# RobotVisionHKA/LiFCal

Measured on AMD Instinct MI355X. Metric: micro-image obs/sec through Jacobian+Schur at 1M obs, higher is better.
Workload: dtype f64; 1 GPU; metric_web: 334 frames, 24720 points, 999994 micro-image observations, window 10, config 0xf06 (2 radial + tangential, mlCenterAdj, Cauchy(0.5), refine poses+points); lens_selection=reference generator (lifcal_mla_project), obs_per_gpu=999994, n_reduced=2021, deterministic=False

## Files before the change

lifcal_amd/csrc/kernels.hpp:

```cpp
#pragma once
#include <hip/hip_runtime.h>
#include <stdint.h>

#include <type_traits>

#include "../../include/lifcal_ba.h"
#include "device_model.hpp"
#include "lm_step.hpp"

namespace lifcal {

constexpr uint32_t DET_NF_MAX = 20;
constexpr int SCAL_COST = 0, SCAL_BAD_U = 1, SCAL_GMAX0 = 2, SCAL_N = 2 + 64;
constexpr int ST_GTD = 0, ST_DDD = 1, ST_STEP2 = 2, ST_X2 = 3, ST_CAND_COST = 4, ST_CHOL_FAIL = 5, ST_GMAX_RED = 6, ST_DIR = 7, ST_N = 8;

struct TileSet { uint32_t n_tiles; const uint32_t *tile_row0, *slot_pt, *slot_fr, *slot_cnt, *ell_lens; const double *ell_u, *ell_v; };

struct Dev {
  uint32_t F, P, Q, NA, bw, nc, n_tiles, n_slots, n_lenses, n_red, ld, M_local, n_owned;
  uint32_t n_radial, tangential, adj, robust, use_poses, use_points, rank, world;
  uint32_t fixed_mask;
  double spx, spy, scale, loss_scale;
  double lm_min, lm_max;
  double *cam, *views, *pts, *cam_c, *views_c, *pts_c;
  const double *lower, *upper;
  CamConsts *camc, *camc_c;
  double *ft, *ft_c, *lt, *lt_c;
  const uint32_t *tile_row0, *slot_pt, *slot_fr, *slot_cnt, *ell_lens;
  const double *ell_u, *ell_v;
  const int32_t* promoted;
  const uint32_t* promoted_ids;
  double* panel_g;
  const uint32_t *pt_slot0, *pt_nslots, *owned;
  const uint8_t* frame_live;
  double *ptacc;
  double *Uinv, *lamP, *sigP;
  double *Wv;
  double *Av;
  const uint8_t* pt_special;
  const uint32_t *gid_fr, *slot_gid;
  uint32_t n_blocks, v2_nfmax, n_special;
  const uint32_t *blk_pass0, *blk_flo, *blk_nf, *pass_pt0, *pass_np, *pass_gid0, *pass_ng, *v2_points, *v2_ptinfo, *v2_slot, *v2_tile_row0, *v2_lens, *v2f_pt, *v2_passpt, *v2_gidx;
  const double *v2_u, *v2_v;
  uint32_t n_fwg;
  const uint32_t *fwg_blk, *fwg_pass0, *blk_pt0;
  const float *v2_du, *v2_dv;
  float* ltf;
  double* ltw;
  uint32_t deterministic, det_stride;
  double *det_slab, *det_slots;
  uint32_t* det_turn;
  const uint32_t* special_owned;
  const uint32_t *c_i, *c_j, *my_cons, *pt_cons0, *pt_cons_list; const double *c_dist, *c_sigma;
  double* Wpart;
  double *Sband, *Sarrow, *rhsacc, *gB, *hdiag, *scal;
  double *sig_red, *lam_red, *delta_red, *Linv;
  double* lm;
  double* step;
  double* dP;
  unsigned long long* dbg;
};

LIFCAL_DEV double lm_radius(const Dev& d, double arg) { return arg < 0.0 ? d.lm[LM_RADIUS] : arg; }

LIFCAL_DEV double* s_addr(const Dev& d, uint32_t row, uint32_t col) {
  if (row < 6 * d.F) {
    const uint32_t f = row / 6, i = row % 6, fc = col / 6, j = col % 6;
    return d.Sband + ((size_t)f * (d.bw + 1) + (f - fc)) * 36 + i * 6 + j;
  }
  return d.Sarrow + (size_t)(row - 6 * d.F) * d.ld + col;
}
LIFCAL_DEV void s_add(const Dev& d, uint32_t row, uint32_t col, double v) {
  if (row >= col) atomicAdd(s_addr(d, row, col), v); else atomicAdd(s_addr(d, col, row), v);
}

LIFCAL_DEV double wave_sum(double v) {
#pragma unroll
  for (int m = 32; m >= 1; m >>= 1) v += __shfl_xor(v, m, 64);
  return v;
}

LIFCAL_DEV void det_turn_wait(const Dev& d, uint32_t which, uint32_t my) {
  uint32_t* turn = d.det_turn + which;
  const uint64_t t0 = __builtin_amdgcn_s_memrealtime();
  for (;;) {
    const uint32_t v = (uint32_t)__builtin_amdgcn_readfirstlane((int)__hip_atomic_load(turn, __ATOMIC_ACQUIRE, __HIP_MEMORY_SCOPE_AGENT));
    if (v == my) break;
    __builtin_amdgcn_s_sleep(16);
// ... 237 lines not shown
  {
    int t = 0;
#pragma unroll
    for (int i = 0; i < NC; ++i) {
#pragma unroll
      for (int j = 0; j <= i; ++j) {
        const double s = wave_sum(cc[t]);
        if (lane == (uint32_t)(t & 63)) { atomicAdd(d.Sarrow + (size_t)(camrow + i) * d.ld + camcol + j, s); if (i == j) atomicAdd(d.hdiag + camcol + i, s); }
        ++t;
      }
    }
#pragma unroll
    for (int i = 0; i < NC; ++i) { const double s = wave_sum(gc[i]); if (lane == (uint32_t)i) atomicAdd(d.gB + camcol + i, s); }
    const double s = wave_sum(cost);
    if (lane == 63) atomicAdd(d.scal + SCAL_COST, s);
  }
  if (d.deterministic) det_turn_pass(d, 0, wave);
}

LIFCAL_DEV double finalize_column(const Dev& d, uint32_t t, double radius) {
  const uint32_t F6 = 6 * d.F, A0 = F6 + 3 * d.Q;
  double* diag = s_addr(d, t, t);
  double* rhs = d.Sarrow + (size_t)d.NA * d.ld;
  const uint32_t fl = t < F6 ? (uint32_t)d.frame_live[t / 6] : 1u;
  const double ch = t >= A0 ? d.camc->chm[t - A0] : 1.0;
  const double s = d.sig_red[t], h = d.hdiag[t], g = d.gB[t], ra = d.rhsacc[t], dg = *diag;
  const double rad = lm_radius(d, radius);
  const bool live = t < F6 ? (d.use_poses && fl) : ch != 0.0;
  const double lam = live ? fmin(fmax(h * s * s, d.lm_min), d.lm_max) / (rad * s * s) : 0.0;
  d.lam_red[t] = lam;
  *diag = live ? dg + lam : 1.0;
  rhs[t] = live ? -g + ra : 0.0;
  return fabs(g);
}

}
#include "sweep2.hpp"
#include "sweep3.hpp"
#include "sweep4.hpp"
namespace lifcal {

__global__ void k_constraints(Dev d, int cost_only, const double* pts, double* cost_out) {
  for (uint32_t t = blockIdx.x * blockDim.x + threadIdx.x; t < d.M_local; t += gridDim.x * blockDim.x) {
  const uint32_t c = d.my_cons[t];
  const uint32_t pi = d.c_i[c], pj = d.c_j[c];
  const double* Pi = pts + 3 * (size_t)pi; const double* Pj = pts + 3 * (size_t)pj;
  const double dx = Pi[0] - Pj[0], dy = Pi[1] - Pj[1], dz = Pi[2] - Pj[2];
  const double n = sqrt(dx * dx + dy * dy + dz * dz);
  const double is = 1.0 / (d.c_sigma[c] + 0.000001);
  const double r = (n - d.c_dist[c]) * is;
  atomicAdd(cost_out, 0.5 * r * r);
  if (cost_only) continue;
  const double in = is / n;
  const double Ji[3] = {dx * in, dy * in, dz * in};
  const uint32_t F6 = 6 * d.F;
  const int32_t qi = d.promoted[pi], qj = d.promoted[pj];
  const uint32_t cj = F6 + 3 * (uint32_t)qj;
  for (int a = 0; a < 3; ++a) {
    for (int b = 0; b <= a; ++b) s_add(d, cj + a, cj + b, Ji[a] * Ji[b]);
    atomicAdd(d.hdiag + cj + a, Ji[a] * Ji[a]);
    atomicAdd(d.gB + cj + a, -Ji[a] * r);
  }
  if (qi < 0) {
    double* acc = d.ptacc + (size_t)pi * 36;
    atomicAdd(acc + 0, Ji[0] * Ji[0]); atomicAdd(acc + 1, Ji[1] * Ji[0]); atomicAdd(acc + 2, Ji[2] * Ji[0]);
    atomicAdd(acc + 3, Ji[1] * Ji[1]); atomicAdd(acc + 4, Ji[2] * Ji[1]); atomicAdd(acc + 5, Ji[2] * Ji[2]);
// ... 279 lines not shown
  const uint32_t e = blockIdx.x, lane = threadIdx.x;
  const uint32_t camrow = 3 * d.Q, camcol = 6 * d.F + 3 * d.Q;
  uint32_t off; double* dst; bool is_max = false;
  if (e < NCC) {
    if (mode != 0) return;
    uint32_t i = 0; while ((i + 1) * (i + 2) / 2 <= e) ++i;
    off = lay.off_cc + e; dst = d.Sarrow + (size_t)(camrow + i) * d.ld + camcol + (e - i * (i + 1) / 2);
  } else if (e < NCC + 3 * NC) {
    const uint32_t q = e - NCC, w = q / NC, j = q % NC;
    if (mode != 0 && w != 1) return;
    off = lay.off_vec + w * vlen + 6 * NFm + j; dst = (w == 0 ? d.gB : (w == 1 ? d.hdiag : d.rhsacc)) + camcol + j;
  } else {
    if (mode != 0) return;
    const uint32_t q = e - NCC - 3 * NC;
    off = lay.off_fr + q; is_max = q == 2;
    dst = d.scal + (q == 0 ? SCAL_COST : (q == 1 ? SCAL_BAD_U : SCAL_GMAX0 + d.rank));
  }
  double v = 0.0;
  for (uint32_t b = lane; b < nB; b += 64) { const double x = d.det_slab[(size_t)b * d.det_stride + off]; v = is_max ? fmax(v, x) : v + x; }
#pragma unroll
  for (int m = 32; m >= 1; m >>= 1) { const double o = __shfl_xor(v, m, 64); v = is_max ? fmax(v, o) : v + o; }
  if (lane == 0) { if (is_max) *dst = fmax(*dst, v); else *dst += v; }
}

__global__ void k_det_sum(const double* slots, uint32_t n_wg, uint32_t K, double* dst) {
  const uint32_t k = threadIdx.x;
  if (k >= K) return;
  double s = 0.0;
  for (uint32_t g = 0; g < n_wg; ++g) s += slots[(size_t)g * K + k];
  dst[k] += s;
}

constexpr uint32_t FIN_ZERO_PER_WG = 256 * 4;
__global__ void k_finalize(Dev d, double radius, uint32_t n_fin, double* zero, uint32_t n_zero) {
  if (blockIdx.x >= n_fin) {
    const uint32_t n_threads = (gridDim.x - n_fin) * blockDim.x, t0 = (blockIdx.x - n_fin) * blockDim.x + threadIdx.x;
    const uint32_t odd = (uint32_t)(((uintptr_t)zero >> 3) & 1u), head = odd < n_zero ? odd : n_zero;
    const uint32_t n2 = (n_zero - head) / 2;
    double2* z2 = reinterpret_cast<double2*>(zero + head);
    for (uint32_t i = t0; i < n2; i += n_threads) z2[i] = double2{0.0, 0.0};
    if (t0 == 0 && head) zero[0] = 0.0;
    if (t0 == 0 && head + 2 * n2 < n_zero) zero[n_zero - 1] = 0.0;
    return;
  }
  const uint32_t t = blockIdx.x * blockDim.x + threadIdx.x;
  if (t == 0) d.lm[LM_T0] = (double)__builtin_amdgcn_s_memrealtime();
  double g = 0.0;
  if (t < d.n_red) g = finalize_column(d, t, radius);
#pragma unroll
  for (int m = 32; m >= 1; m >>= 1) g = fmax(g, __shfl_xor(g, m, 64));
  if ((threadIdx.x & 63u) == 0) atomicMax((unsigned long long*)(d.step + ST_GMAX_RED), (unsigned long long)__double_as_longlong(g));
}

__global__ __launch_bounds__(1024) void k_band_chol(Dev d) {
  extern __shared__ __attribute__((aligned(16))) double smem[];
  double* Ld = smem; double* Li = smem + 36; double* failp = smem + 72;
  double* panel = d.panel_g ? d.panel_g : smem + 80;
  const uint32_t tid = threadIdx.x, nt = blockDim.x;
  const uint32_t F = d.F, bw = d.bw, NAx = d.NA + 1, ld = d.ld;
  if (tid == 0) *failp = 0.0;
  __syncthreads();
  for (uint32_t j = 0; j < F; ++j) {
    double* Sjj = d.Sband + (size_t)j * (bw + 1) * 36;
    if (tid == 0) {
      double L[6][6];
      for (int a = 0; a < 6; ++a) for (int b = 0; b <= a; ++b) L[a][b] = Sjj[a * 6 + b];
      bool ok = true;
      for (int c = 0; c < 6; ++c) {
        double dg = L[c][c];
        for (int k = 0; k < c; ++k) dg -= L[c][k] * L[c][k];
        if (!(dg > 0.0)) { ok = false; dg = 1.0; }
        dg = sqrt(dg); L[c][c] = dg;
        for (int r = c + 1; r < 6; ++r) { double s = L[r][c]; for (int k = 0; k < c; ++k) s -= L[r][k] * L[c][k]; L[r][c] = s / dg; }
      }
      if (!ok) *failp = 1.0;
      double I[6][6];
      for (int c = 0; c < 6; ++c) {
        for (int r = 0; r < 6; ++r) I[r][c] = 0.0;
        I[c][c] = 1.0 / L[c][c];
        for (int r = c + 1; r < 6; ++r) { double s = 0.0; for (int k = c; k < r; ++k) s -= L[r][k] * I[k][c]; I[r][c] = s / L[r][r]; }
      }
      for (int a = 0; a < 6; ++a) for (int b = 0; b < 6; ++b) { Ld[a * 6 + b] = (b <= a) ? L[a][b] : 0.0; Li[a * 6 + b] = (b <= a) ? I[a][b] : 0.0; }
      for (int a = 0; a < 6; ++a) for (int b = 0; b <= a; ++b) Sjj[a * 6 + b] = L[a][b];
      for (int k = 0; k < 36; ++k) d.Linv[(size_t)j * 36 + k] = Li[k];
    }
// ... 491 lines not shown
```

lifcal_amd/csrc/lifcal_ba.hip:

```cpp
#include <hip/hip_runtime.h>
#include <hip/hip_ext.h>

#include <dlfcn.h>

#include <chrono>
#include <cmath>
#include <cstdio>
#include <cstdlib>
#include <cstring>
#include <limits>
#include <mutex>
#include <string>
#include <vector>

#include "../../include/lifcal_ba.h"
#include "kernels.hpp"
#include "plan.hpp"
#include "linesearch.hpp"
#include "sweep_state.hpp"

using namespace lifcal;

static_assert(lifcal::DET_NF_MAX == lifcal::Plan::NF_MAX, "k_det_reduce searches the covering blocks of a frame inside Plan::NF_MAX frames");
static_assert(lifcal::Plan::PASS_GROUPS == 256, "k_det_reduce / k_det_reduce_all read the window layout of 256-lane passes (V2Lds(nf, true, 256))");
// ... 115 lines not shown
  std::vector<hipEvent_t> prof_events; uint32_t prof_cap = 0, prof_used = 0, prof_seen = 0, prof_stride = 1; bool prof_on = false, prof_closed = false;
  hipEvent_t prof_span0 = nullptr, prof_span1 = nullptr;
  hipEvent_t prof_ev(int which) { return prof_events[(size_t)prof_used * 6 + which]; }
  bool prof_in_span() const { return prof_on && prof_seen < prof_cap; }
  bool prof_active() const { return prof_in_span() && prof_seen % prof_stride == 0; }
};

namespace {

template <class T>
int dev_alloc(lifcal_ba_handle* h, T** p, size_t n) {
  *p = nullptr;
  if (n == 0) n = 1;
  HIP_TRY(hipMalloc((void**)p, n * sizeof(T)));
  h->allocs.push_back(*p);
  h->bytes += n * sizeof(T);
  return 0;
}
template <class T, class A>
int dev_upload(lifcal_ba_handle* h, T** p, const std::vector<T, A>& v) {
  if (int rc = dev_alloc(h, p, v.size())) return rc;
  if (!v.empty()) HIP_TRY(hipMemcpy(*p, v.data(), v.size() * sizeof(T), hipMemcpyHostToDevice));
  return 0;
}

int do_allreduce(lifcal_ba_handle* h, double* buf, size_t count) {
  if (h->opt.world_size <= 1) return 0;
  if (h->hook) { if (h->hook(h->hook_ctx, buf, count, (void*)h->stream) != 0) { g_last_error = "all-reduce hook failed"; return LIFCAL_BA_ERR_COMM; } return 0; }
  if (h->comm) { if (g_rccl.AllReduce(buf, buf, count, kNcclFloat64, kNcclSum, h->comm, h->stream) != 0) { g_last_error = "ncclAllReduce failed"; return LIFCAL_BA_ERR_COMM; } return 0; }
  g_last_error = "world_size > 1 but neither lifcal_ba_set_allreduce nor lifcal_ba_comm_init_rccl was called";
  return LIFCAL_BA_ERR_COMM;
}

int exchange_reduced(lifcal_ba_handle* h) {
  if (h->opt.world_size <= 1 && !h->force_exchange) return 0;
  const bool have_gather = h->ghook ? (h->hook != nullptr) : (h->hook == nullptr && h->comm != nullptr);
  if (!h->xch_ok || !have_gather) return do_allreduce(h, h->red_block, h->red_count);
  const Xch& x = h->xch;
  hipLaunchKernelGGL(k_xch_pack, dim3((x.SL + 255) / 256), dim3(256), 0, h->stream, h->d, x);
  HIP_TRY(hipGetLastError());
  if (h->ghook) {
    if (h->ghook(h->ghook_ctx, x.send, (void*)x.recv, x.SL, (void*)h->stream) != 0) { g_last_error = "all-gather hook failed"; return LIFCAL_BA_ERR_COMM; }
  } else if (g_rccl.AllGather(x.send, (void*)x.recv, x.SL, kNcclFloat64, h->comm, h->stream) != 0) {
    h->xch_ok = false;
    return do_allreduce(h, h->red_block, h->red_count);
  }
  const size_t n = (size_t)(x.F6 / 6) * x.BS + (size_t)x.NA * x.F6 + (size_t)3 * x.F6 + x.NA * x.NA + 3 * x.NA + SCAL_N;
  hipLaunchKernelGGL(k_xch_unpack, dim3((unsigned)((n + 255) / 256)), dim3(256), 0, h->stream, h->d, x);
  HIP_TRY(hipGetLastError());
  return 0;
}

#ifdef LIFCAL_ONLY_FULL_CFG
#define DISPATCH_CFG(h, CALL) do { if ((h)->plan.n_radial == 2 && (h)->plan.tangential && (h)->plan.adj) { CALL(2, true, true); } else { g_last_error = "development build: configuration not compiled in"; return LIFCAL_BA_ERR_INVALID_ARG; } } while (0)
#define DISPATCH_LENS(h, CALL) do { if ((h)->plan.n_radial == 2 && (h)->plan.tangential) { CALL(2, true); } else { g_last_error = "development build: configuration not compiled in"; return LIFCAL_BA_ERR_INVALID_ARG; } } while (0)
#else
#define DISPATCH_CFG(h, CALL)                                                       \
  do {                                                                              \
    const int nr_ = (h)->plan.n_radial; const bool tn_ = (h)->plan.tangential, aj_ = (h)->plan.adj; \
    if (nr_ == 0 && !tn_ && !aj_) { CALL(0, false, false); }                        \
    else if (nr_ == 0 && !tn_ && aj_) { CALL(0, false, true); }                     \
    else if (nr_ == 0 && tn_ && !aj_) { CALL(0, true, false); }                     \
    else if (nr_ == 0 && tn_ && aj_) { CALL(0, true, true); }                       \
    else if (nr_ == 1 && !tn_ && !aj_) { CALL(1, false, false); }                   \
    else if (nr_ == 1 && !tn_ && aj_) { CALL(1, false, true); }                     \
    else if (nr_ == 1 && tn_ && !aj_) { CALL(1, true, false); }                     \
    else if (nr_ == 1 && tn_ && aj_) { CALL(1, true, true); }                       \
    else if (nr_ == 2 && !tn_ && !aj_) { CALL(2, false, false); }                   \
// ... 20 lines not shown

int launch_tables(lifcal_ba_handle* h, const double* cam, const double* views, CamConsts* camc, double* ft, double* lt, bool tangents, bool fold, float* ltf = nullptr) {
  const Dev& d = h->d;
  const uint32_t grid = std::max(1u, (std::max(d.n_lenses, d.F) + 255) / 256);
#define CALL_TABLES(NR, TAN) hipLaunchKernelGGL((k_tables<NR, TAN>), dim3(grid), dim3(256), 0, h->stream, d, cam, views, camc, ft, lt, (const double*)h->lens_xy, tangents ? 1 : 0, fold ? 1 : 0, ltf)
  DISPATCH_LENS(h, CALL_TABLES);
#undef CALL_TABLES
  HIP_TRY(hipGetLastError());
  return 0;
}

int ensure_current_tables(lifcal_ba_handle* h) {
  Dev& d = h->d;
  if (!ss_sweep_needs_tables(&h->ss)) return 0;
  if (int rc = launch_tables(h, d.cam, d.views, d.camc, d.ft, d.lt, true, true, d.ltf)) return rc;
  ss_tables_built(&h->ss, SS_CURRENT, SS_CURRENT, true, true);
  return 0;
}
int build_candidate_tables(lifcal_ba_handle* h) {
  Dev& d = h->d;
  if (int rc = launch_tables(h, d.cam_c, d.views_c, d.camc_c, d.ft_c, d.lt_c, true, true)) return rc;
  ss_tables_built(&h->ss, SS_CANDIDATE, SS_CANDIDATE, true, true);
  return 0;
}
int build_stats_tables(lifcal_ba_handle* h) {
  Dev& d = h->d;
  ss_tables_clobbered(&h->ss, SS_CANDIDATE);
  return launch_tables(h, d.cam, d.views, h->camc_stats, d.ft_c, d.lt_c, false, false);
}

void bind_block(lifcal_ba_handle* h, int which) {
  Dev& d = h->d;
  const size_t n_band = (size_t)d.F * (d.bw + 1) * 36, n_arrow = (size_t)(d.NA + 1) * d.ld;
  h->red_block = h->red_blocks[which];
  d.Sband = h->red_block; d.Sarrow = d.Sband + n_band; d.rhsacc = d.Sarrow + n_arrow; d.gB = d.rhsacc + d.n_red; d.hdiag = d.gB + d.n_red; d.scal = d.hdiag + d.n_red;
  d.step = d.scal + SCAL_N; h->partial = d.step + ST_N;
}
int acquire_block(lifcal_ba_handle* h) {
  const bool fill = ss_acquire_block(&h->ss);
  bind_block(h, h->ss.bound);
  if (fill) HIP_TRY(hipMemsetAsync(h->red_block, 0, (h->red_count + ST_N) * sizeof(double), h->stream));
  return 0;
}

void launch_constraints(lifcal_ba_handle* h, int cost_only, const double* pts, double* out) {
  const Dev& d = h->d;
  if (d.M_local) hipLaunchKernelGGL(k_constraints, dim3(d.deterministic ? 1 : (d.M_local + 63) / 64), dim3(d.deterministic ? 1 : 64), 0, h->stream, d, cost_only, pts, out);
}

int launch_value_cost(lifcal_ba_handle* h, const CamConsts* camc, const double* ft, const double* lt, const double* pts, double* out) {
  const Dev& d = h->d;
  for (const TileSet* ts : {&h->ts1, &h->ts2}) {
    if (!ts->n_tiles) continue;
    const uint32_t grid = std::max(1u, std::min((ts->n_tiles + 3) / 4, 1024u));
#define CALL_COST(NR, TAN, ADJ) hipLaunchKernelGGL((k_cost<NR, TAN, ADJ>), dim3(grid), dim3(256), 0, h->stream, d, *ts, camc, ft, lt, pts, out)
    DISPATCH_CFG(h, CALL_COST);
#undef CALL_COST
    if (d.deterministic) hipLaunchKernelGGL(k_det_sum, dim3(1), dim3(64), 0, h->stream, (const double*)d.det_slots, grid, 1u, out);
  }
  launch_constraints(h, 1, pts, out);
  HIP_TRY(hipGetLastError());
  return 0;
}

int launch_blocks(lifcal_ba_handle* h, double radius, int mode) {
  if (int rc = acquire_block(h)) return rc;
  Dev& d = h->d;
  if (d.n_special) hipLaunchKernelGGL(k_zero_special, dim3((d.n_special * 36 + 255) / 256), dim3(256), 0, h->stream, d);
  if (d.deterministic && (d.n_tiles || d.n_special)) HIP_TRY(hipMemsetAsync(d.det_turn, 0, 4 * sizeof(uint32_t), h->stream));
  const bool prof = mode == 0 && h->prof_active();
  hipEvent_t ev_a = prof ? h->prof_ev(1) : nullptr, ev_b = prof ? h->prof_ev(2) : nullptr;
  if (d.n_blocks && h->use_sweep4) {
#define CALL_FRONT4(NR, TAN, ADJ) hipExtLaunchKernelGGL((k_front4<NR, TAN, ADJ>), dim3(d.n_fwg), dim3(F4_THREADS), h->f4_lds, h->stream, ev_a, mode == 0 ? nullptr : ev_b, 0, d, mode)
    DISPATCH_CFG(h, CALL_FRONT4);
#undef CALL_FRONT4
    if (mode == 0) {
#define CALL_BACK4(NCV) do { if (h->b4_tpt == 1) hipExtLaunchKernelGGL((k_back4<NCV, 1>), dim3(d.n_blocks), dim3(B4_THREADS), h->b4_lds, h->stream, nullptr, ev_b, 0, d, radius); \
                             else hipExtLaunchKernelGGL((k_back4<NCV, 2>), dim3(d.n_blocks), dim3(B4_THREADS), h->b4_lds, h->stream, nullptr, ev_b, 0, d, radius); } while (0)
      switch (d.nc) { case 5: CALL_BACK4(5); break; case 6: CALL_BACK4(6); break; case 7: CALL_BACK4(7); break; case 8: CALL_BACK4(8); break; default: CALL_BACK4(9); break; }
#undef CALL_BACK4
    }
  } else if (d.n_blocks) {
    hipEvent_t ev_stop = d.deterministic ? nullptr : ev_b;
#define LAUNCH_DOM(KERNEL, THREADS) hipExtLaunchKernelGGL(KERNEL, dim3(d.n_blocks), dim3(THREADS), h->v2_lds_bytes, h->stream, ev_a, ev_stop, 0, d, radius, mode)
#define CALL_SWEEP2(NR, TAN, ADJ) LAUNCH_DOM((k_sweep2<NR, TAN, ADJ>), 256)
#define CALL_SWEEP3(NR, TAN, ADJ) LAUNCH_DOM((k_sweep3<NR, TAN, ADJ, 4>), 512)
#define CALL_SWEEP3F(NR, TAN, ADJ) LAUNCH_DOM((k_sweep3<NR, TAN, ADJ, 4, float>), 512)
#define CALL_SWEEP3H(NR, TAN, ADJ) LAUNCH_DOM((k_sweep3<NR, TAN, ADJ, 2>), 256)
    if (h->opt.precision == 1) DISPATCH_CFG(h, CALL_SWEEP3F);
    else if (h->use_sweep3 && h->sweep_waves == 2) DISPATCH_CFG(h, CALL_SWEEP3H); else if (h->use_sweep3) DISPATCH_CFG(h, CALL_SWEEP3); else DISPATCH_CFG(h, CALL_SWEEP2);
#undef CALL_SWEEP3H
#undef CALL_SWEEP3F
    if (d.deterministic) {
// ... 12 lines not shown
#define CALL_SWEEP(NR, TAN, ADJ) hipLaunchKernelGGL((k_sweep<NR, TAN, ADJ>), dim3(sweep_grid(h)), dim3(256), 0, h->stream, d)
    DISPATCH_CFG(h, CALL_SWEEP);
#undef CALL_SWEEP
  }
  if (prof && !d.n_blocks) HIP_TRY(hipEventRecord(ev_b, h->stream));
  launch_constraints(h, 0, d.pts, d.scal + SCAL_COST);
  if (d.Q && d.use_points) hipLaunchKernelGGL(k_promote_diag, dim3((d.Q + 63) / 64), dim3(64), 0, h->stream, d);
  HIP_TRY(hipGetLastError());
  return 0;
}

int launch_sweep(lifcal_ba_handle* h, double radius) {
  Dev& d = h->d;
  h->swept = false;
  if (h->prof_in_span() && h->prof_seen == 0) HIP_TRY(hipEventRecord(h->prof_span0, h->stream));
  if (int rc = ensure_current_tables(h)) return rc;
  if (!h->sigma_valid) {
    if (int rc = launch_blocks(h, radius, 1)) return rc;
    const double* hd = d.hdiag;
    if (h->opt.world_size > 1) {
      HIP_TRY(hipMemcpyAsync(h->hdiag_tmp, d.hdiag, d.n_red * sizeof(double), hipMemcpyDeviceToDevice, h->stream));
      if (int rc = do_allreduce(h, h->hdiag_tmp, d.n_red)) return rc;
      hd = h->hdiag_tmp;
    }
    Dev dj = d; dj.hdiag = const_cast<double*>(hd);
    const uint32_t n = std::max(d.n_red, d.P);
    hipLaunchKernelGGL(k_jacobi, dim3((n + 255) / 256), dim3(256), 0, h->stream, dj, h->opt.jacobi_scaling ? 1 : 0);
    HIP_TRY(hipGetLastError());
    h->sigma_valid = true;
  }
  if (int rc = launch_blocks(h, radius, 0)) return rc;
  if (d.use_points && d.n_special) hipLaunchKernelGGL(k_schur, dim3((d.n_special + 3) / 4), dim3(256), 0, h->stream, d, radius);
  HIP_TRY(hipGetLastError());
  {
    const bool prof_x = h->prof_active() && (h->opt.world_size > 1 || h->force_exchange);
    if (prof_x) HIP_TRY(hipEventRecord(h->prof_ev(3), h->stream));
    if (int rc = exchange_reduced(h)) return rc;
    if (prof_x) HIP_TRY(hipEventRecord(h->prof_ev(4), h->stream));
  }
  {
    const uint32_t n_fin = (d.n_red + 255) / 256;
    const uint32_t n_zero = (uint32_t)(h->red_count + ST_N);
    const uint32_t n_fill = std::min((n_zero + FIN_ZERO_PER_WG - 1) / FIN_ZERO_PER_WG, 1024u);
    hipLaunchKernelGGL(k_finalize, dim3(n_fin + n_fill), dim3(256), 0, h->stream, d, radius, n_fin, h->red_blocks[h->ss.bound ^ 1], n_zero);
    HIP_TRY(hipGetLastError());
    ss_finalize_cleaned_other(&h->ss);
  }
  if (h->prof_in_span()) {
    if (h->prof_seen + 1 == h->prof_cap) { HIP_TRY(hipEventRecord(h->prof_span1, h->stream)); h->prof_closed = true; }
    if (h->prof_active()) h->prof_used++;
    h->prof_seen++;
  }
  return 0;
}

int read_sweep_scalars(lifcal_ba_handle* h, double* cost, double* gmax, double* bad_u) {
  Dev& d = h->d;
  HIP_TRY(hipMemcpyAsync(h->h_scal, d.scal, (SCAL_N + ST_N) * sizeof(double), hipMemcpyDeviceToHost, h->stream));
  HIP_TRY(hipStreamSynchronize(h->stream));
  *cost = h->h_scal[SCAL_COST];
  *bad_u = h->h_scal[SCAL_BAD_U];
  double g = 0.0;
  for (int r = 0; r < 64; ++r) { double v; std::memcpy(&v, &h->h_scal[SCAL_GMAX0 + r], 8); if (v > g) g = v; }
  double gr; std::memcpy(&gr, &h->h_scal[SCAL_N + ST_GMAX_RED], 8);
  *gmax = std::max(g, gr);
  return 0;
}

int launch_linear_solve(lifcal_ba_handle* h) {
  Dev& d = h->d;
  if (h->use_cr) {
    const CrSys sys{d.Sband, d.Sarrow, d.delta_red, d.step + ST_CHOL_FAIL, d.F, d.bw, d.NA, d.ld};
    cr_solve_launch(h->cr, sys, h->stream);
  } else if (h->bandw_ok && h->twisted) {
    const uint32_t m = h->tw_m, bw = d.bw, n2 = d.F - m - bw;
    const BandSeg sa{+1, 0u, m + bw, m, 0u, h->dumpA}, sb{-1, d.F - 1, n2 + bw, n2, 0u, h->dumpB}, sm{+1, m, bw, bw, 1u, nullptr};
    hipLaunchKernelGGL(k_band_chol_seg, dim3(2), dim3(256), h->bandw_lds, h->stream, d, h->Lpanel, sa, sb);
// ... 41 lines not shown
void swap_current_candidate(lifcal_ba_handle* h) {
  Dev& d = h->d;
  std::swap(d.cam, d.cam_c); std::swap(d.views, d.views_c);
  if (d.use_points) std::swap(d.pts, d.pts_c);
  ss_swap_parameters(&h->ss);
}
void accept_candidate(lifcal_ba_handle* h) {
  Dev& d = h->d;
  const bool with_tables = h->opt.precision == 0;
  std::swap(d.cam, d.cam_c); std::swap(d.views, d.views_c);
  if (d.use_points) std::swap(d.pts, d.pts_c);
  if (with_tables) { std::swap(d.camc, d.camc_c); std::swap(d.ft, d.ft_c); std::swap(d.lt, d.lt_c); }
  ss_host_accept(&h->ss, with_tables);
}

int launch_apply_step(lifcal_ba_handle* h, double t) {
  Dev& d = h->d;
  HIP_TRY(hipMemsetAsync(h->ls_buf, 0, 8 * sizeof(double), h->stream));
  const uint32_t n = std::max(std::max(6 * d.F, 17u), std::max(d.n_owned, d.Q));
  hipLaunchKernelGGL(k_apply_step, dim3((n + 255) / 256), dim3(256), 0, h->stream, d, t, h->ls_buf);
  ss_candidate_written(&h->ss);
  if (d.deterministic) hipLaunchKernelGGL(k_det_sum, dim3(1), dim3(64), 0, h->stream, (const double*)d.det_slots, (n + 255) / 256, 2u, h->ls_buf);
  HIP_TRY(hipGetLastError());
  return 0;
}

int eval_trial(lifcal_ba_handle* h, double t, double radius, LsSample* smp) {
  Dev& d = h->d;
  if (int rc = launch_apply_step(h, t)) return rc;
  swap_current_candidate(h);
  int rc = ensure_current_tables(h);
  if (!rc) rc = launch_blocks(h, radius, 0);
  if (!rc && d.use_points && d.n_special) { hipLaunchKernelGGL(k_schur, dim3((d.n_special + 3) / 4), dim3(256), 0, h->stream, d, radius); }
  if (!rc) rc = do_allreduce(h, h->red_block, h->red_count);
  if (!rc) {
    const uint32_t n = std::max(d.n_red, d.n_owned);
    hipLaunchKernelGGL(k_dirderiv, dim3((n + 255) / 256), dim3(256), 0, h->stream, d, h->ls_buf + 2);
    if (d.deterministic) hipLaunchKernelGGL(k_det_sum, dim3(1), dim3(64), 0, h->stream, (const double*)d.det_slots, (n + 255) / 256, 1u, h->ls_buf + 2);
    if (hipGetLastError() != hipSuccess) rc = LIFCAL_BA_ERR_HIP;
  }
  const bool value64 = h->opt.precision == 1;
  if (!rc && value64) rc = launch_value_cost(h, d.camc, d.ft, d.lt, d.pts, h->ls_buf + 3);
  swap_current_candidate(h);
  if (rc) return rc;
  if (int rc2 = do_allreduce(h, h->ls_buf, value64 ? 4 : 3)) return rc2;
  double hb[8], cost;
  HIP_TRY(hipMemcpyAsync(hb, h->ls_buf, sizeof(hb), hipMemcpyDeviceToHost, h->stream));
  HIP_TRY(hipMemcpyAsync(&cost, d.scal + SCAL_COST, sizeof(double), hipMemcpyDeviceToHost, h->stream));
  HIP_TRY(hipStreamSynchronize(h->stream));
  if (value64) cost = hb[3];
  smp->x = t; smp->value = cost; smp->value_valid = std::isfinite(cost);
  smp->gradient = hb[2]; smp->gradient_valid = smp->value_valid && std::isfinite(smp->gradient);
  return 0;
}

struct StepScalars { double gtd, ddd, step2, x2, cand_cost, chol_fail; };

int read_step_scalars(lifcal_ba_handle* h, StepScalars* s) {
  HIP_TRY(hipMemcpyAsync(h->h_scal, h->d.step, (ST_N + 8) * sizeof(double), hipMemcpyDeviceToHost, h->stream));
  HIP_TRY(hipStreamSynchronize(h->stream));
  const double* p = h->h_scal + ST_N;
  *s = {p[0], p[1], p[2], p[3], p[4], h->h_scal[ST_CHOL_FAIL]};
  return 0;
}

int step_dir_max(lifcal_ba_handle* h, double* dir_max) {
// ... 413 lines not shown
    }
    blk_pt0[L.n_blocks] = (uint32_t)L.v2_points.size();
    fwg_pass0.push_back(L.n_passes);
    d.n_fwg = (uint32_t)fwg_blk.size();
    if (cclk.on) std::fprintf(stderr, "[create] k_front4: %d workgroups per CU (occupancy API), %u workgroups over %u blocks, LDS %zu B; k_back4: LDS %zu B, %d tile(s) per thread\n",
                              per_cu, d.n_fwg, d.n_blocks, h->f4_lds, h->b4_lds, h->b4_tpt);
    { uint32_t* t; U(t, fwg_blk); d.fwg_blk = t; U(t, fwg_pass0); d.fwg_pass0 = t; U(t, blk_pt0); d.blk_pt0 = t; }
  } else if (d.n_blocks) {
#define SET_LDS(NR, TAN, ADJ) do { if (hipFuncSetAttribute((const void*)k_sweep2<NR, TAN, ADJ>, hipFuncAttributeMaxDynamicSharedMemorySize, (int)h->v2_lds_bytes) != hipSuccess) return fail(LIFCAL_BA_ERR_HIP); \
    if (hipFuncSetAttribute((const void*)k_sweep3<NR, TAN, ADJ, 4>, hipFuncAttributeMaxDynamicSharedMemorySize, (int)h->v2_lds_bytes) != hipSuccess) return fail(LIFCAL_BA_ERR_HIP); \
    if (hipFuncSetAttribute((const void*)k_sweep3<NR, TAN, ADJ, 2>, hipFuncAttributeMaxDynamicSharedMemorySize, (int)h->v2_lds_bytes) != hipSuccess) return fail(LIFCAL_BA_ERR_HIP); \
    if (hipFuncSetAttribute((const void*)k_sweep3<NR, TAN, ADJ, 4, float>, hipFuncAttributeMaxDynamicSharedMemorySize, (int)h->v2_lds_bytes) != hipSuccess) return fail(LIFCAL_BA_ERR_HIP); } while (0)
    DISPATCH_CFG(h, SET_LDS);
#undef SET_LDS
  }
  { double* t; U(t, L.ell_u); d.ell_u = t; U(t, L.ell_v); d.ell_v = t; }
  h->ts1 = TileSet{d.n_tiles, d.tile_row0, d.slot_pt, d.slot_fr, d.slot_cnt, d.ell_lens, d.ell_u, d.ell_v};
  { int32_t* t; U(t, L.promoted); d.promoted = t; }
  { uint32_t* t; U(t, L.promoted_ids); d.promoted_ids = t; U(t, L.pt_slot0); d.pt_slot0 = t; U(t, L.pt_nslots); d.pt_nslots = t; U(t, L.owned_points); d.owned = t; }
  { std::vector<uint8_t> live(L.frame_used); uint8_t* t; U(t, live); d.frame_live = t; h->frame_live_dev = t; h->frame_live_host = live; }
  A(d.ptacc, (size_t)d.P * 36); A(d.Uinv, (size_t)d.P * 9);
  if (hipMemset(d.ptacc, 0, (size_t)std::max(1u, d.P) * 36 * sizeof(double)) != hipSuccess) return fail(LIFCAL_BA_ERR_HIP); A(d.lamP, (size_t)d.P * 3); A(d.sigP, (size_t)d.P * 3);
  A(d.Wv, (size_t)L.n_groups * 18);
  A(d.Av, (size_t)L.n_groups * 6);
  { uint8_t* t; U(t, L.pt_special); d.pt_special = t; }
  if (L.use_constraints) {
    uint32_t* t; U(t, L.c_i); d.c_i = t; U(t, L.c_j); d.c_j = t; U(t, L.my_constraints); d.my_cons = t;
    U(t, L.pt_cons0); d.pt_cons0 = t; U(t, L.pt_cons_list); d.pt_cons_list = t;
    double* f; U(f, L.c_dist); d.c_dist = f; U(f, L.c_sigma); d.c_sigma = f;
    A(d.Wpart, (size_t)L.M * 9);
  }
  const size_t n_band = (size_t)d.F * (d.bw + 1) * 36, n_arrow = (size_t)(d.NA + 1) * d.ld;
  h->red_count = n_band + n_arrow + 3 * (size_t)d.n_red + SCAL_N;
  A(h->red_blocks[0], h->red_count + ST_N + 8); A(h->red_blocks[1], h->red_count + ST_N + 8);
  ss_reset(&h->ss);
  bind_block(h, h->ss.bound);
  A(d.sig_red, d.n_red); A(d.lam_red, d.n_red); A(d.delta_red, d.n_red); A(d.Linv, (size_t)d.F * 36 + 36);
  h->force_exchange = getenv("LIFCAL_FORCE_EXCHANGE") != nullptr;
  if ((opt.world_size > 1 || h->force_exchange) && d.Q == 0 && d.use_poses && getenv("LIFCAL_DENSE_ALLREDUCE") == nullptr) {
    Xch& x = h->xch;
    x.world = (uint32_t)opt.world_size; x.rank = (uint32_t)opt.rank; x.BS = (d.bw + 1) * 36; x.NA = d.NA; x.F6 = 6 * d.F;
    uint32_t maxn = 1;
    for (uint32_t n : L.rk_nfr) maxn = std::max(maxn, n);
    x.maxn = maxn;
    const uint64_t off_arrow = (uint64_t)maxn * x.BS, off_vec = off_arrow + (uint64_t)maxn * x.NA * 6, off_tail = off_vec + (uint64_t)maxn * 18;
    const uint64_t SL = off_tail + (uint64_t)x.NA * x.NA + 3 * x.NA + SCAL_N;
    if (SL < (1ull << 31) && (uint64_t)x.world * SL <= 2 * (uint64_t)h->red_count) {
      x.off_arrow = (uint32_t)off_arrow; x.off_vec = (uint32_t)off_vec; x.off_tail = (uint32_t)off_tail; x.SL = (uint32_t)SL;
      uint32_t* t; U(t, L.rk_flo); x.flo = t; U(t, L.rk_nfr); x.nfr = t;
      double* b; A(b, (size_t)SL); x.send = b; A(b, (size_t)x.world * SL); x.recv = b;
      h->xch_ok = true;
    }
  }
  A(d.dbg, std::max((size_t)std::max(1u, d.n_blocks) * 32, (size_t)d.n_fwg * 64));
  A(d.dP, 3 * (size_t)d.P); A(h->ls_buf, 8); A(h->dirmax_buf, 65); A(d.lm, LM_N);
  A(h->hdiag_tmp, d.n_red); A(h->stats_buf, 8); A(h->stats_slots, 4 + 2 * 64); A(h->pts_gather, 3 * (size_t)d.P);
  const size_t panel_rows = 6 * (size_t)d.bw + d.NA + 1;
  const size_t lds_need = (80 + panel_rows * 6) * sizeof(double);
  if (lds_need <= 64 * 1024) { h->chol_lds = lds_need; d.panel_g = nullptr; }
  else { h->chol_lds = 80 * sizeof(double); A(d.panel_g, panel_rows * 6); }
  {
    const BandLds bl(d.bw, d.NA);
    h->bandw_lds = (size_t)bl.total * sizeof(double);
    h->backw_lds = (size_t)std::max(1u, d.n_red) * sizeof(double);
    h->bandw_ok = h->bandw_lds <= 160 * 1024 && h->backw_lds <= 160 * 1024 && getenv("LIFCAL_DISABLE_BANDW") == nullptr;
    if (h->bandw_ok) {
      A(h->Lpanel, (size_t)std::max(1u, d.F) * (6 * (size_t)d.bw + d.NA + 1) * 6);
// ... 468 lines not shown
```

lifcal_amd/csrc/sweep3.hpp:

```cpp
#pragma once

namespace lifcal {

template <int NR, bool TAN, bool ADJ, int WR, class ET = double>
__global__ __launch_bounds__(128 * WR, 2) void k_sweep3(Dev d, double radius, int mode) {
  constexpr bool F32 = sizeof(ET) == 4;
  constexpr int NC = 5 + NR + (TAN ? 2 : 0);
  constexpr int NCC = NC * (NC + 1) / 2;
  constexpr int HV = 6 + 2 * NC + 2;
  constexpr uint32_t LP = 64u * WR;
  constexpr uint32_t NT = 2u * LP;
  static_assert(HV * LP <= V2Lds::zd_for(LP), "hand-off buffer must fit the Z matrix");
  if (radius < 0.0 && d.lm[LM_TERMINATION] != 0.0) return;
  extern __shared__ __attribute__((aligned(16))) double sm[];
  const V2Lds lay(d.v2_nfmax, true, LP);
  const uint32_t NFm = lay.nfm, vlen = 6 * NFm + NCMAX + 3;
  double* Spp = sm; double* Scp = sm + lay.off_cp; double* Scc = sm + lay.off_cc;
  double* vgB = sm + lay.off_vec; double* vhd = vgB + vlen; double* vrhs = vhd + vlen;
  double* Fr = sm + lay.off_fr;
  double* slab = sm + lay.off_slab;
  double* Zd = sm + lay.off_zd;
  double* misc = sm + lay.off_misc;
  uint32_t* pidl = (uint32_t*)(misc + MISC_DOUBLES);
  unsigned short* colinfo = (unsigned short*)(misc + MISC_DOUBLES + 32);
// ... 633 lines not shown
    }
    constexpr int NVB = NCC + NC;
    constexpr uint32_t NROWS = 4u * WR;
    {
      double* red = Zd;
      const uint32_t rowi = t256 >> 4;
      const bool tail = (lane & 15u) == 15u;
#pragma unroll
      for (int idx = 0; idx < NVB; ++idx) {
        double v = (idx < NCC) ? cc[idx < NCC ? idx : 0] : gc[(idx - NCC) >= 0 && (idx - NCC) < NC ? idx - NCC : 0];
        v = dpp_add_step<0x111, 0xf>(v); v = dpp_add_step<0x112, 0xf>(v); v = dpp_add_step<0x114, 0xf>(v); v = dpp_add_step<0x118, 0xf>(v);
        if (tail) red[rowi * NVB + idx] = v;
      }
      lds_barrier();
      if (t256 < (uint32_t)NVB) {
        const int idx = (int)t256;
        double sacc = 0.0;
#pragma unroll
        for (uint32_t k = 0; k < NROWS; ++k) sacc += red[k * NVB + idx];
        if (idx < NCC) {
          int i = 0; while ((i + 1) * (i + 2) / 2 <= idx) ++i;
          if (mode == 0) Scc[idx] += sacc;
          if (idx == i * (i + 1) / 2 + i) vhd[6 * NFm + i] += sacc;
        } else {
          vgB[6 * NFm + (idx - NCC)] += sacc;
        }
      }
      lds_barrier();
    }
  }
  lds_barrier();
  STAMP(10);
  if (!det) {
    const uint32_t F6 = 6 * d.F, camrow = 3 * d.Q, camcol = F6 + 3 * d.Q;
    if (mode == 0 && tid < (uint32_t)NCC) {
      uint32_t i = 0; while ((i + 1) * (i + 2) / 2 <= tid) ++i;
      const uint32_t j = tid - i * (i + 1) / 2;
      atomicAdd(d.Sarrow + (size_t)(camrow + i) * d.ld + camcol + j, Scc[tid]);
    }
    if (tid < (uint32_t)NC) {
      atomicAdd(d.hdiag + camcol + tid, vhd[6 * NFm + tid]);
      if (mode == 0) { atomicAdd(d.gB + camcol + tid, vgB[6 * NFm + tid]); atomicAdd(d.rhsacc + camcol + tid, vrhs[6 * NFm + tid]); }
    }
    if (mode == 0 && tid == 0) {
      atomicAdd(d.scal + SCAL_COST, misc[0]);
      if (misc[1] != 0.0) atomicAdd(d.scal + SCAL_BAD_U, misc[1]);
      atomicMax((unsigned long long*)(d.scal + SCAL_GMAX0 + d.rank), *(unsigned long long*)(misc + 2));
    }
  }
  for (uint32_t i = tid; i < FRV * nf; i += NT) {
    const uint32_t v = i / nf, lf = i % nf;
    double sacc = 0.0;
    for (uint32_t r = 0; r < lay.nrep; ++r) sacc += Fr[(size_t)v * NFm * lay.nrep + r * NFm + lf];
    if (v < 21) {
      uint32_t a = 0; while ((a + 1) * (a + 2) / 2 <= v) ++a;
      const uint32_t bb = v - a * (a + 1) / 2;
      Spp[(size_t)(lf * (lf + 1) / 2 + lf) * 36 + a * 6 + bb] += sacc;
      if (a == bb) vhd[6 * lf + a] += sacc;
    } else if (v < 27) {
      vgB[6 * lf + (v - 21)] += sacc;
    } else if (mode == 0 && v < 27 + 6 * (uint32_t)NC) {
      const uint32_t j = (v - 27) / 6, ci = (v - 27) % 6;
      Scp[(size_t)j * 6 * NFm + 6 * lf + ci] += sacc;
    }
  }
  lds_barrier();
  STAMP(11);
  if (det) {
    double* out = d.det_slab + (size_t)b * d.det_stride;
    for (uint32_t i = tid; i < lay.off_fr; i += NT) out[i] = sm[i];
    if (tid < 3) out[lay.off_fr + tid] = misc[tid];
    return;
  }
  const uint32_t F6 = 6 * d.F, camrow = 3 * d.Q, camcol = F6 + 3 * d.Q;
  for (uint32_t i = tid; i < 6 * nf; i += NT) atomicAdd(d.hdiag + 6 * flo + i, vhd[i]);
  if (mode == 0) {
    for (uint32_t i = tid; i < 6 * nf; i += NT) { atomicAdd(d.gB + 6 * flo + i, vgB[i]); atomicAdd(d.rhsacc + 6 * flo + i, vrhs[i]); }
    for (uint32_t i = tid; i < (uint32_t)NC * 6 * nf; i += NT) {
      const uint32_t j = i / (6 * nf), cidx = i % (6 * nf);
      atomicAdd(d.Sarrow + (size_t)(camrow + j) * d.ld + 6 * flo + cidx, Scp[(size_t)j * 6 * NFm + cidx]);
    }
    const uint32_t npp = nf * (nf + 1) / 2;
    for (uint32_t i = tid; i < npp * 36; i += NT) {
      const uint32_t blk = i / 36, e = i % 36;
      uint32_t a = (uint32_t)((sqrtf(8.0f * (float)blk + 1.0f) - 1.0f) * 0.5f);
      while (a * (a + 1) / 2 > blk) --a;
      while ((a + 1) * (a + 2) / 2 <= blk) ++a;
      const uint32_t bb = blk - a * (a + 1) / 2, dd = a - bb;
      const double v = Spp[i];
      if (dd <= d.bw && v != 0.0 && !(dd == 0 && (e % 6) > (e / 6))) atomicAdd(d.Sband + ((size_t)(flo + a) * (d.bw + 1) + dd) * 36 + e, v);
    }
  }
#ifdef LIFCAL_STAMPS
  lds_barrier();
  STAMP(5);
  if ((tid == 0 || tid == LP) && d.dbg) for (int i = 0; i < 16; ++i) d.dbg[(size_t)b * 32 + (tid == 0 ? 0 : 16) + i] = st_acc[i];
#endif
}

}
```

Measured before the change: 9.658 billion obs/s.

## Spread camera-block atomics across eight hot rows and fold them in finalize

Every workgroup of the sweep3 kernel used to atomically add its camera-camera Schur block, camera gradient/diagonal/rhs terms, cost and gradient max into the same global words, which serialises contention on a few cache lines. Those contributions now go to one of eight padded 'hot' rows chosen by block index. The rows are summed into the real targets by a dedicated block inside the finalize kernel, or by a small separate kernel before a multi-rank exchange. The cost is extra memory to zero and a fold step that must run before the camera columns are finalized.

```diff
diff --git a/lifcal_amd/csrc/kernels.hpp b/lifcal_amd/csrc/kernels.hpp
--- a/lifcal_amd/csrc/kernels.hpp
+++ b/lifcal_amd/csrc/kernels.hpp
@@ -12,6 +12,8 @@
 
 constexpr uint32_t DET_NF_MAX = 20;
 constexpr int SCAL_COST = 0, SCAL_BAD_U = 1, SCAL_GMAX0 = 2, SCAL_N = 2 + 64;
+constexpr uint32_t HOT_ROWS = 8, HOT_STRIDE = 80, HOT_N = HOT_ROWS * HOT_STRIDE;
+static_assert(NCMAX * (NCMAX + 1) / 2 + 3 * NCMAX + 2 <= HOT_STRIDE && HOT_STRIDE % 16 == 0, "a row holds every hot word and is a whole number of 128-byte lines");
 constexpr int ST_GTD = 0, ST_DDD = 1, ST_STEP2 = 2, ST_X2 = 3, ST_CAND_COST = 4, ST_CHOL_FAIL = 5, ST_GMAX_RED = 6, ST_DIR = 7, ST_N = 8;
 
 struct TileSet { uint32_t n_tiles; const uint32_t *tile_row0, *slot_pt, *slot_fr, *slot_cnt, *ell_lens; const double *ell_u, *ell_v; };
@@ -54,6 +56,7 @@
   const uint32_t *c_i, *c_j, *my_cons, *pt_cons0, *pt_cons_list; const double *c_dist, *c_sigma;
   double* Wpart;
   double *Sband, *Sarrow, *rhsacc, *gB, *hdiag, *scal;
+  double* hot;
   double *sig_red, *lam_red, *delta_red, *Linv;
   double* lm;
   double* step;
@@ -357,6 +360,37 @@
   *diag = live ? dg + lam : 1.0;
   rhs[t] = live ? -g + ra : 0.0;
   return fabs(g);
+}
+
+LIFCAL_DEV void fold_hot_rows(const Dev& d, uint32_t w) {
+  const uint32_t NC = d.nc, NCC = NC * (NC + 1) / 2, nw = NCC + 3 * NC + 2;
+  if (w >= nw) return;
+  double v[HOT_ROWS];
+#pragma unroll
+  for (uint32_t r = 0; r < HOT_ROWS; ++r) v[r] = d.hot[r * HOT_STRIDE + w];
+  const uint32_t camrow = 3 * d.Q, camcol = 6 * d.F + 3 * d.Q;
+  if (w == nw - 1) {
+    unsigned long long* dst = (unsigned long long*)(d.scal + SCAL_GMAX0 + d.rank);
+    unsigned long long m = *dst;
+#pragma unroll
+    for (uint32_t r = 0; r < HOT_ROWS; ++r) { const unsigned long long x = (unsigned long long)__double_as_longlong(v[r]); m = x > m ? x : m; }
+    *dst = m;
+    return;
+  }
+  double* dst;
+  if (w < NCC) {
+    uint32_t i = 0; while ((i + 1) * (i + 2) / 2 <= w) ++i;
+    dst = d.Sarrow + (size_t)(camrow + i) * d.ld + camcol + (w - i * (i + 1) / 2);
+  } else if (w < NCC + 3 * NC) {
+    const uint32_t q = w - NCC, vec = q / NC;
+    dst = (vec == 0 ? d.hdiag : (vec == 1 ? d.gB : d.rhsacc)) + camcol + q % NC;
+  } else {
+    dst = d.scal + SCAL_COST;
+  }
+  double s = 0.0;
+#pragma unroll
+  for (uint32_t r = 0; r < HOT_ROWS; ++r) s += v[r];
+  *dst += s;
 }
 
 }
@@ -702,7 +736,7 @@
 }
 
 constexpr uint32_t FIN_ZERO_PER_WG = 256 * 4;
-__global__ void k_finalize(Dev d, double radius, uint32_t n_fin, double* zero, uint32_t n_zero) {
+__global__ void k_finalize(Dev d, double radius, uint32_t n_fin, double* zero, uint32_t n_zero, uint32_t fold) {
   if (blockIdx.x >= n_fin) {
     const uint32_t n_threads = (gridDim.x - n_fin) * blockDim.x, t0 = (blockIdx.x - n_fin) * blockDim.x + threadIdx.x;
     const uint32_t odd = (uint32_t)(((uintptr_t)zero >> 3) & 1u), head = odd < n_zero ? odd : n_zero;
@@ -713,14 +747,24 @@
     if (t0 == 0 && head + 2 * n2 < n_zero) zero[n_zero - 1] = 0.0;
     return;
   }
-  const uint32_t t = blockIdx.x * blockDim.x + threadIdx.x;
-  if (t == 0) d.lm[LM_T0] = (double)__builtin_amdgcn_s_memrealtime();
+  const uint32_t A0 = 6 * d.F + 3 * d.Q;
   double g = 0.0;
-  if (t < d.n_red) g = finalize_column(d, t, radius);
+  if (fold && blockIdx.x == 0) {
+    if (threadIdx.x == 0) d.lm[LM_T0] = (double)__builtin_amdgcn_s_memrealtime();
+    fold_hot_rows(d, threadIdx.x);
+    __syncthreads();
+    if (A0 + threadIdx.x < d.n_red) g = finalize_column(d, A0 + threadIdx.x, radius);
+  } else {
+    const uint32_t t = (blockIdx.x - fold) * blockDim.x + threadIdx.x;
+    if (!fold && t == 0) d.lm[LM_T0] = (double)__builtin_amdgcn_s_memrealtime();
+    if (t < (fold ? A0 : d.n_red)) g = finalize_column(d, t, radius);
+  }
 #pragma unroll
   for (int m = 32; m >= 1; m >>= 1) g = fmax(g, __shfl_xor(g, m, 64));
   if ((threadIdx.x & 63u) == 0) atomicMax((unsigned long long*)(d.step + ST_GMAX_RED), (unsigned long long)__double_as_longlong(g));
 }
+
+__global__ __launch_bounds__(256) void k_fold_hot(Dev d) { fold_hot_rows(d, threadIdx.x); }
 
 __global__ __launch_bounds__(1024) void k_band_chol(Dev d) {
   extern __shared__ __attribute__((aligned(16))) double smem[];
diff --git a/lifcal_amd/csrc/lifcal_ba.hip b/lifcal_amd/csrc/lifcal_ba.hip
--- a/lifcal_amd/csrc/lifcal_ba.hip
+++ b/lifcal_amd/csrc/lifcal_ba.hip
@@ -171,8 +171,10 @@
   return LIFCAL_BA_ERR_COMM;
 }
 
+bool exchanges(const lifcal_ba_handle* h) { return h->opt.world_size > 1 || h->force_exchange; }
+
 int exchange_reduced(lifcal_ba_handle* h) {
-  if (h->opt.world_size <= 1 && !h->force_exchange) return 0;
+  if (!exchanges(h)) return 0;
   const bool have_gather = h->ghook ? (h->hook != nullptr) : (h->hook == nullptr && h->comm != nullptr);
   if (!h->xch_ok || !have_gather) return do_allreduce(h, h->red_block, h->red_count);
   const Xch& x = h->xch;
@@ -259,14 +261,14 @@
 void bind_block(lifcal_ba_handle* h, int which) {
   Dev& d = h->d;
   const size_t n_band = (size_t)d.F * (d.bw + 1) * 36, n_arrow = (size_t)(d.NA + 1) * d.ld;
-  h->red_block = h->red_blocks[which];
+  d.hot = h->red_blocks[which]; h->red_block = d.hot + HOT_N;
   d.Sband = h->red_block; d.Sarrow = d.Sband + n_band; d.rhsacc = d.Sarrow + n_arrow; d.gB = d.rhsacc + d.n_red; d.hdiag = d.gB + d.n_red; d.scal = d.hdiag + d.n_red;
   d.step = d.scal + SCAL_N; h->partial = d.step + ST_N;
 }
 int acquire_block(lifcal_ba_handle* h) {
   const bool fill = ss_acquire_block(&h->ss);
   bind_block(h, h->ss.bound);
-  if (fill) HIP_TRY(hipMemsetAsync(h->red_block, 0, (h->red_count + ST_N) * sizeof(double), h->stream));
+  if (fill) HIP_TRY(hipMemsetAsync(h->d.hot, 0, (HOT_N + h->red_count + ST_N) * sizeof(double), h->stream));
   return 0;
 }
 
@@ -286,6 +288,16 @@
     if (d.deterministic) hipLaunchKernelGGL(k_det_sum, dim3(1), dim3(64), 0, h->stream, (const double*)d.det_slots, grid, 1u, out);
   }
   launch_constraints(h, 1, pts, out);
+  HIP_TRY(hipGetLastError());
+  return 0;
+}
+
+bool uses_hot_rows(const lifcal_ba_handle* h) {
+  return h->d.n_blocks && !h->d.deterministic && !h->use_sweep4 && (h->opt.precision == 1 || h->use_sweep3);
+}
+int launch_fold_hot(lifcal_ba_handle* h) {
+  if (!uses_hot_rows(h)) return 0;
+  hipLaunchKernelGGL(k_fold_hot, dim3(1), dim3(256), 0, h->stream, h->d);
   HIP_TRY(hipGetLastError());
   return 0;
 }
@@ -364,17 +376,20 @@
   if (int rc = launch_blocks(h, radius, 0)) return rc;
   if (d.use_points && d.n_special) hipLaunchKernelGGL(k_schur, dim3((d.n_special + 3) / 4), dim3(256), 0, h->stream, d, radius);
   HIP_TRY(hipGetLastError());
+  const bool exchanged = exchanges(h);
   {
-    const bool prof_x = h->prof_active() && (h->opt.world_size > 1 || h->force_exchange);
+    const bool prof_x = h->prof_active() && exchanged;
+    if (exchanged) { if (int rc = launch_fold_hot(h)) return rc; }
     if (prof_x) HIP_TRY(hipEventRecord(h->prof_ev(3), h->stream));
     if (int rc = exchange_reduced(h)) return rc;
     if (prof_x) HIP_TRY(hipEventRecord(h->prof_ev(4), h->stream));
   }
   {
-    const uint32_t n_fin = (d.n_red + 255) / 256;
-    const uint32_t n_zero = (uint32_t)(h->red_count + ST_N);
+    const uint32_t fold = !exchanged && uses_hot_rows(h) ? 1u : 0u;
+    const uint32_t n_fin = (fold ? (d.n_red - d.nc + 255) / 256 + 1 : (d.n_red + 255) / 256);
+    const uint32_t n_zero = (uint32_t)(HOT_N + h->red_count + ST_N);
     const uint32_t n_fill = std::min((n_zero + FIN_ZERO_PER_WG - 1) / FIN_ZERO_PER_WG, 1024u);
-    hipLaunchKernelGGL(k_finalize, dim3(n_fin + n_fill), dim3(256), 0, h->stream, d, radius, n_fin, h->red_blocks[h->ss.bound ^ 1], n_zero);
+    hipLaunchKernelGGL(k_finalize, dim3(n_fin + n_fill), dim3(256), 0, h->stream, d, radius, n_fin, h->red_blocks[h->ss.bound ^ 1], n_zero, fold);
     HIP_TRY(hipGetLastError());
     ss_finalize_cleaned_other(&h->ss);
   }
@@ -482,6 +497,7 @@
   int rc = ensure_current_tables(h);
   if (!rc) rc = launch_blocks(h, radius, 0);
   if (!rc && d.use_points && d.n_special) { hipLaunchKernelGGL(k_schur, dim3((d.n_special + 3) / 4), dim3(256), 0, h->stream, d, radius); }
+  if (!rc) rc = launch_fold_hot(h);
   if (!rc) rc = do_allreduce(h, h->red_block, h->red_count);
   if (!rc) {
     const uint32_t n = std::max(d.n_red, d.n_owned);
@@ -961,7 +977,7 @@
   }
   const size_t n_band = (size_t)d.F * (d.bw + 1) * 36, n_arrow = (size_t)(d.NA + 1) * d.ld;
   h->red_count = n_band + n_arrow + 3 * (size_t)d.n_red + SCAL_N;
-  A(h->red_blocks[0], h->red_count + ST_N + 8); A(h->red_blocks[1], h->red_count + ST_N + 8);
+  A(h->red_blocks[0], HOT_N + h->red_count + ST_N + 8); A(h->red_blocks[1], HOT_N + h->red_count + ST_N + 8);
   ss_reset(&h->ss);
   bind_block(h, h->ss.bound);
   A(d.sig_red, d.n_red); A(d.lam_red, d.n_red); A(d.delta_red, d.n_red); A(d.Linv, (size_t)d.F * 36 + 36);
diff --git a/lifcal_amd/csrc/sweep3.hpp b/lifcal_amd/csrc/sweep3.hpp
--- a/lifcal_amd/csrc/sweep3.hpp
+++ b/lifcal_amd/csrc/sweep3.hpp
@@ -689,20 +689,21 @@
   lds_barrier();
   STAMP(10);
   if (!det) {
-    const uint32_t F6 = 6 * d.F, camrow = 3 * d.Q, camcol = F6 + 3 * d.Q;
-    if (mode == 0 && tid < (uint32_t)NCC) {
-      uint32_t i = 0; while ((i + 1) * (i + 2) / 2 <= tid) ++i;
-      const uint32_t j = tid - i * (i + 1) / 2;
-      atomicAdd(d.Sarrow + (size_t)(camrow + i) * d.ld + camcol + j, Scc[tid]);
-    }
-    if (tid < (uint32_t)NC) {
-      atomicAdd(d.hdiag + camcol + tid, vhd[6 * NFm + tid]);
-      if (mode == 0) { atomicAdd(d.gB + camcol + tid, vgB[6 * NFm + tid]); atomicAdd(d.rhsacc + camcol + tid, vrhs[6 * NFm + tid]); }
-    }
-    if (mode == 0 && tid == 0) {
-      atomicAdd(d.scal + SCAL_COST, misc[0]);
-      if (misc[1] != 0.0) atomicAdd(d.scal + SCAL_BAD_U, misc[1]);
-      atomicMax((unsigned long long*)(d.scal + SCAL_GMAX0 + d.rank), *(unsigned long long*)(misc + 2));
+    if (mode == 0) {
+      double* hr = d.hot + (size_t)(b % HOT_ROWS) * HOT_STRIDE;
+      if (tid < (uint32_t)NCC) atomicAdd(hr + tid, Scc[tid]);
+      if (tid < (uint32_t)NC) {
+        atomicAdd(hr + NCC + tid, vhd[6 * NFm + tid]);
+        atomicAdd(hr + NCC + NC + tid, vgB[6 * NFm + tid]);
+        atomicAdd(hr + NCC + 2 * NC + tid, vrhs[6 * NFm + tid]);
+      }
+      if (tid == 0) {
+        atomicAdd(hr + NCC + 3 * NC, misc[0]);
+        if (misc[1] != 0.0) atomicAdd(d.scal + SCAL_BAD_U, misc[1]);
+        atomicMax((unsigned long long*)(hr + NCC + 3 * NC + 1), *(unsigned long long*)(misc + 2));
+      }
+    } else if (tid < (uint32_t)NC) {
+      atomicAdd(d.hdiag + 6 * d.F + 3 * d.Q + tid, vhd[6 * NFm + tid]);
     }
   }
   for (uint32_t i = tid; i < FRV * nf; i += NT) {
@@ -729,7 +730,7 @@
     if (tid < 3) out[lay.off_fr + tid] = misc[tid];
     return;
   }
-  const uint32_t F6 = 6 * d.F, camrow = 3 * d.Q, camcol = F6 + 3 * d.Q;
+  const uint32_t camrow = 3 * d.Q;
   for (uint32_t i = tid; i < 6 * nf; i += NT) atomicAdd(d.hdiag + 6 * flo + i, vhd[i]);
   if (mode == 0) {
     for (uint32_t i = tid; i < 6 * nf; i += NT) { atomicAdd(d.gB + 6 * flo + i, vgB[i]); atomicAdd(d.rhsacc + 6 * flo + i, vrhs[i]); }
```

Measured after the change: 9.882 billion obs/s (median of 6 runs). 2.3% higher.
